# EndlessReform/smoltts

Hardware: AMD Instinct MI355X
Metric: Mimi frames/sec (=12.5 x RTF), greedy DualAR decode + Mimi decode to PCM (higher is better)
Workload: dtype bf16 weights, fp32 activations/accumulate, fp32 KV cache (LM); fp32 (Mimi)

## Files before the change

smoltts_amd/csrc/conv_xs.hip:

```cpp
#include <stdlib.h>

#include "gemm_dev.h"

namespace smoltts {

namespace {

constexpr int XS_RA_CONV = 80;
constexpr int XS_MAX_CIN = 256, XS_MAX_K_LINEAR = 512;

__device__ __forceinline__ float elu_hw_xs(float x) { return x > 0.f ? x : __expf(x) - 1.0f; }

#ifdef SMOLTTS_DBG_XS_STAMPS
__device__ unsigned long long g_xs_stamps[8 * 8];
#define XS_STAMP(I) { const long long now_ = clock64(); st_sum[I] += now_ - st_last; st_last = now_; }
#else
#define XS_STAMP(I)
#endif

template <int NTW, int MT, int RA, int EPI, int NP>
__global__ __launch_bounds__(512) void conv_xs_kernel(GemmDev p) {
  constexpr int XS_S = 16 * MT, XS_MT = MT, XS_RA = RA;
  extern __shared__ __attribute__((aligned(16))) uint4 xp[];
  const int tid = threadIdx.x, lane = tid & 63;
  const int wave = __builtin_amdgcn_readfirstlane(tid >> 6);
  const int r = lane & 15, q = lane >> 4;
  const int b = blockIdx.y, row0 = blockIdx.x * XS_S, T = p.rows_per_batch > 0 ? p.rows_per_batch : p.M;
  const int G = p.cpt * 4, nrows = XS_S + p.taps - 1, nchunks = p.K >> 5;
  const int kz = p.ksplit > 1 ? (int)blockIdx.z : 0;
  const int nt0 = (p.ksplit > 1 ? 0 : (int)blockIdx.z * 8 * NTW) + wave * NTW;
  const int nloc = p.ksplit > 1 ? p.cpt : nchunks;
  const float* xb = p.x + (long)b * p.x_bstride + (long)row0 * p.ldx + (long)kz * p.cpt * 32;
#ifdef SMOLTTS_DBG_XS_STAMPS
  long long st_sum[6] = {0, 0, 0, 0, 0, 0}, st_last = clock64();
#endif

  if (p.ln_w != nullptr) {
    float4 va[4][2];
    float* psum = reinterpret_cast<float*>(xp + 3 * G * XS_RA);
    float* stat = psum + 32 * 64;
#pragma unroll
    for (int it = 0; it < 4; ++it) {
      const int idx = tid + 512 * it, i = idx / (8 * G) * 8 + (idx & 7), g8 = (idx >> 3) % G;
      va[it][0] = va[it][1] = make_float4(0.f, 0.f, 0.f, 0.f);
      if (row0 + i < T) {
        const float* src = xb + (long)i * p.ldx + g8 * 8;
        va[it][0] = *reinterpret_cast<const float4*>(src);
        va[it][1] = *reinterpret_cast<const float4*>(src + 4);
      }
      const float4 a = va[it][0], c = va[it][1];
      psum[i * 64 + g8] = ((a.x + a.y) + (a.z + a.w)) + ((c.x + c.y) + (c.z + c.w));
    }
    lds_barrier();
    const int srow = tid >> 4, l16 = tid & 15;
    {
      const float4 t = *reinterpret_cast<const float4*>(psum + srow * 64 + l16 * 4);
      float sm = (t.x + t.y) + (t.z + t.w);
      sm += __shfl_xor(sm, 8); sm += __shfl_xor(sm, 4); sm += __shfl_xor(sm, 2); sm += __shfl_xor(sm, 1);
      if (l16 == 0) stat[srow] = sm / (float)p.K;
    }
    lds_barrier();
#pragma unroll
    for (int it = 0; it < 4; ++it) {
      const int idx = tid + 512 * it, i = idx / (8 * G) * 8 + (idx & 7), g8 = (idx >> 3) % G;
      const float mu = stat[i];
      const float4 a = va[it][0], c = va[it][1];
      float v = 0.f;
      v = fmaf(a.x - mu, a.x - mu, v); v = fmaf(a.y - mu, a.y - mu, v); v = fmaf(a.z - mu, a.z - mu, v); v = fmaf(a.w - mu, a.w - mu, v);
      v = fmaf(c.x - mu, c.x - mu, v); v = fmaf(c.y - mu, c.y - mu, v); v = fmaf(c.z - mu, c.z - mu, v); v = fmaf(c.w - mu, c.w - mu, v);
      psum[i * 64 + g8] = v;
    }
    lds_barrier();
    {
      const float4 t = *reinterpret_cast<const float4*>(psum + srow * 64 + l16 * 4);
      float sm = (t.x + t.y) + (t.z + t.w);
      sm += __shfl_xor(sm, 8); sm += __shfl_xor(sm, 4); sm += __shfl_xor(sm, 2); sm += __shfl_xor(sm, 1);
      if (l16 == 0) stat[32 + srow] = 1.0f / sqrtf(sm / (float)p.K + p.eps);
    }
    lds_barrier();
#pragma unroll
    for (int it = 0; it < 4; ++it) {
      const int idx = tid + 512 * it, i = idx / (8 * G) * 8 + (idx & 7), g8 = (idx >> 3) % G;
      const float mu = stat[i], rs = stat[32 + i];
      const float4 w0 = *reinterpret_cast<const float4*>(p.ln_w + g8 * 8), w1 = *reinterpret_cast<const float4*>(p.ln_w + g8 * 8 + 4);
      const float4 b0 = *reinterpret_cast<const float4*>(p.ln_b + g8 * 8), b1 = *reinterpret_cast<const float4*>(p.ln_b + g8 * 8 + 4);
      float4 a = va[it][0], c = va[it][1];
      a = make_float4((a.x - mu) * rs * w0.x + b0.x, (a.y - mu) * rs * w0.y + b0.y, (a.z - mu) * rs * w0.z + b0.z, (a.w - mu) * rs * w0.w + b0.w);
      c = make_float4((c.x - mu) * rs * w1.x + b1.x, (c.y - mu) * rs * w1.y + b1.y, (c.z - mu) * rs * w1.z + b1.z, (c.w - mu) * rs * w1.w + b1.w);
      uint4 h, m, l;
      split3x8(a, c, h, m, l);
      const int slot = g8 * XS_RA + i;
      xp[slot] = h;
      xp[slot + G * XS_RA] = m;
      xp[slot + 2 * G * XS_RA] = l;
    }
  } else
  for (int idx = tid; idx < ((nrows + 7) & ~7) * G; idx += 512) {
    const int i = idx / (8 * G) * 8 + (idx & 7), g8 = (idx >> 3) % G;
    if (i >= nrows) continue;
    float4 a = make_float4(0.f, 0.f, 0.f, 0.f), c = a;
    if (row0 + i < T + p.taps - 1) {
      const float* src = xb + (long)i * p.ldx + g8 * 8;
      a = *reinterpret_cast<const float4*>(src);
      c = *reinterpret_cast<const float4*>(src + 4);
    }
    if (p.pro_elu) {
      a = make_float4(elu_hw_xs(a.x), elu_hw_xs(a.y), elu_hw_xs(a.z), elu_hw_xs(a.w));
      c = make_float4(elu_hw_xs(c.x), elu_hw_xs(c.y), elu_hw_xs(c.z), elu_hw_xs(c.w));
    }
    uint4 h, m, l;
    split3x8(a, c, h, m, l);
    const int slot = g8 * XS_RA + i;
    xp[slot] = h;
    xp[slot + G * XS_RA] = m;
    xp[slot + 2 * G * XS_RA] = l;
  }

  XS_STAMP(0)
  f32x4 acc[XS_MT][NTW];
#pragma unroll
  for (int mt = 0; mt < XS_MT; ++mt)
#pragma unroll
    for (int t = 0; t < NTW; ++t) acc[mt][t] = (f32x4){0.f, 0.f, 0.f, 0.f};

  const char* wtile = p.w3 + ((size_t)nt0 * nchunks + (size_t)kz * p.cpt) * 3072;
  const int wlane = lane * 16;
  uint4 wq[2][NTW][3];
#pragma unroll
  for (int t = 0; t < NTW; ++t)
#pragma unroll
    for (int pc = 0; pc < 3; ++pc) wq[0][t][pc] = *reinterpret_cast<const uint4*>(wtile + (size_t)(t * nchunks) * 3072 + pc * 1024 + wlane);
  lds_barrier();
  XS_STAMP(1)

  int tap = 0, xc = 0;
#define XS_CHUNK(BUF, KC)                                                                                               \
  {                                                                                                                     \
    if ((KC) + 1 < nloc) {                                                                                              \
      _Pragma("unroll") for (int t = 0; t < NTW; ++t)                                                                   \
        _Pragma("unroll") for (int pc = 0; pc < 3; ++pc)                                                                \
          wq[(BUF) ^ 1][t][pc] = *reinterpret_cast<const uint4*>(wtile + (size_t)(t * nchunks + (KC) + 1) * 3072 + pc * 1024 + wlane); \
    }                                                                                                                   \
    __builtin_amdgcn_sched_barrier(0);  \
    _Pragma("unroll") for (int mt = 0; mt < XS_MT; ++mt) {                                                              \
      uint4 xf[3];                                                                                                      \
      _Pragma("unroll") for (int pc = 0; pc < 3; ++pc) xf[pc] = xp[(pc * G + xc * 4 + q) * XS_RA + mt * 16 + r + tap];  \
      _Pragma("unroll") for (int t = 0; t < NTW; ++t) acc[mt][t] = mfma_b3<NP>(wq[BUF][t], xf, acc[mt][t]);                \
    }                                                                                                                   \
    if (++xc == p.cpt) { xc = 0; ++tap; }                                                                               \
  }
  int kc = 0;
  for (; kc + 1 < nloc; kc += 2) {
    XS_CHUNK(0, kc)
    XS_CHUNK(1, kc + 1)
  }
  if (kc < nloc) XS_CHUNK(0, kc)
#undef XS_CHUNK
  XS_STAMP(2)

  if (EPI == SMOLTTS_EPI_RESID && p.ksplit <= 1 && (p.N & 15) == 0) {
    float4 rr[XS_MT][NTW];
#pragma unroll
    for (int mt = 0; mt < XS_MT; ++mt) {
      const int rl = row0 + mt * 16 + r;
#pragma unroll
      for (int t = 0; t < NTW; ++t) {
        rr[mt][t] = make_float4(0.f, 0.f, 0.f, 0.f);
        if (rl < T) rr[mt][t] = *reinterpret_cast<const float4*>(p.resid + row_off(b * T + rl, p.rows_per_batch, p.ldr, p.r_bstride) + (nt0 + t) * 16 + q * 4);
      }
    }
#pragma unroll
    for (int mt = 0; mt < XS_MT; ++mt) {
      const int rl = row0 + mt * 16 + r;
      if (rl >= T) continue;
      const long orow = row_off(b * T + rl, p.rows_per_batch, p.ldo, p.o_bstride);
#pragma unroll
      for (int t = 0; t < NTW; ++t) {
        float v[4] = {acc[mt][t][0], acc[mt][t][1], acc[mt][t][2], acc[mt][t][3]};
        rows_epilogue_resid(p, orow, (nt0 + t) * 16 + q * 4, v, rr[mt][t]);
      }
    }
  } else {
#pragma unroll
  for (int mt = 0; mt < XS_MT; ++mt) {
    const int rl = row0 + mt * 16 + r;
    if (rl >= T) continue;
    const int m = b * T + rl;
    const long orow = row_off(m, p.rows_per_batch, p.ldo, p.o_bstride);
#pragma unroll
    for (int t = 0; t < NTW; ++t) {
      const int n0 = (nt0 + t) * 16 + q * 4;
      if (p.ksplit > 1) {
        *reinterpret_cast<float4*>(p.splitk_ws + ((long)kz * p.M + m) * p.N + n0) = make_float4(acc[mt][t][0], acc[mt][t][1], acc[mt][t][2], acc[mt][t][3]);
        continue;
      }
      float v[4] = {acc[mt][t][0], acc[mt][t][1], acc[mt][t][2], acc[mt][t][3]};
      rows_epilogue<EPI>(p, m, orow, n0, v);
    }
  }
  }
#ifdef SMOLTTS_DBG_XS_STAMPS
  XS_STAMP(3)
  if (tid == 0) {
    const int st_row = p.ksplit > 1 ? 6 : (EPI == 0 && NTW == 1) ? 2 : EPI;
    for (int i = 0; i < 4; ++i) atomicAdd(&g_xs_stamps[st_row * 8 + i], (unsigned long long)st_sum[i]);
    atomicAdd(&g_xs_stamps[st_row * 8 + 6], 1ull);
  }
#endif
}

template <int NTW, int MT, int RA, int EPI, int NP>
int launch_xs_np(const GemmDev& g, int nsplit, hipStream_t stream) {
  const size_t lds = (size_t)3 * (g.cpt * 4) * RA * 16 + (g.ln_w ? (32 * 64 + 64) * sizeof(float) : 0);
  static PerDevice attr;
  const int dev = PerDevice::current();
  if (!attr.done(dev) || (int)lds > attr.value[dev]) {
    ST_CHECK_HIP(hipFuncSetAttribute((const void*)conv_xs_kernel<NTW, MT, RA, EPI, NP>, hipFuncAttributeMaxDynamicSharedMemorySize, (int)lds));
    if ((int)lds > attr.value[dev]) attr.value[dev] = (int)lds;
    attr.mark_done(dev);
  }
  const int T = g.rows_per_batch > 0 ? g.rows_per_batch : g.M;
  const dim3 grid((T + 16 * MT - 1) / (16 * MT), g.M / T, nsplit);
  hipLaunchKernelGGL((conv_xs_kernel<NTW, MT, RA, EPI, NP>), grid, dim3(512), lds, stream, g);
  ST_CHECK_HIP(hipGetLastError());
  return SMOLTTS_OK;
}

template <int NTW, int MT, int RA, int EPI>
int launch_xs(const GemmDev& g, int nsplit, hipStream_t stream) {
  return g.b3_products == 3 ? launch_xs_np<NTW, MT, RA, EPI, 3>(g, nsplit, stream) : launch_xs_np<NTW, MT, RA, EPI, 6>(g, nsplit, stream);
}

bool linear_ksplit(const GemmDev& d, int epilogue) {
  return epilogue == SMOLTTS_EPI_SCALE_RESID && d.N == 512 && d.K == 2048 && d.splitk_ws && 4L * d.M * d.N <= d.splitk_cap;
}

int linear_ntw(const GemmDev& d, int epilogue) {
  if (d.rows_per_batch > 0) {
    if (epilogue == SMOLTTS_EPI_RESID && d.K <= 256 && (d.N == 256 || d.N == 512)) return d.N / 128;
    return 0;
  }
  if (epilogue == SMOLTTS_EPI_QKV_ROPE && d.N == 1536) return 3;
  if (epilogue == SMOLTTS_EPI_SCALE_RESID && d.N == 512) return 1;
  if (epilogue == SMOLTTS_EPI_GELU && d.N == 2048) return 4;
  return 0;
}

}

bool conv_xs_applies(const GemmDev& d, int epilogue) {
  static const bool off = ST_KNOB_INT("SMOLTTS_CONV_XS", 1) == 0;
  static const bool lin_off = ST_KNOB_INT("SMOLTTS_LINEAR_XS", 1) == 0;
  if (off || !d.w3) return false;
  if (d.x_bstride % 4 != 0 || d.ldo % 4 != 0 || d.o_bstride % 4 != 0 || d.ldx % 4 != 0) return false;
  if (d.ldx >= d.K && linear_ksplit(d, epilogue)) {
    if (lin_off || d.pro_elu || d.ln_w) return false;
    const int T = d.rows_per_batch > 0 ? d.rows_per_batch : d.M;
    return d.M % T == 0 && d.M / T <= 65535 && (long)((T + 31) / 32) * (d.M / T) * 4 >= 256;
  }
  if (d.ldx >= d.K) {
    if (lin_off || d.pro_elu || d.K > XS_MAX_K_LINEAR || d.K % 32 != 0 || linear_ntw(d, epilogue) == 0) return false;
    if (d.ln_w && (d.rows_per_batch > 0 || d.K != 512 || !d.ln_b)) return false;
    if (d.rows_per_batch > 0)
      return d.M % d.rows_per_batch == 0 && d.M / d.rows_per_batch <= 65535 && (long)((d.rows_per_batch + 63) / 64) * (d.M / d.rows_per_batch) >= 256;
    return (long)((d.M + 31) / 32) * 4 >= 256;
  }
  if (d.ln_w || epilogue != SMOLTTS_EPI_STORE || d.rows_per_batch <= 0 || d.M % d.rows_per_batch != 0) return false;
  if (d.ldx % 32 != 0 || d.ldx > XS_MAX_CIN || d.K % d.ldx != 0) return false;
  const int taps = (int)(d.K / d.ldx);
  if (taps < 2 || 64 + taps - 1 > XS_RA_CONV || (d.N != 128 && d.N != 640)) return false;
  const long tiles = (long)((d.rows_per_batch + 63) / 64) * (d.M / d.rows_per_batch);
  return tiles >= 256 && d.M / d.rows_per_batch <= 65535;
}

int launch_conv_xs(const GemmDev& d, int epilogue, hipStream_t stream) {
  GemmDev g = d;
  if (d.ldx >= d.K && linear_ksplit(d, epilogue)) {
    g.taps = 1;
    g.cpt = 16;
    g.ksplit = 4;
    ST_TRY((launch_xs<4, 2, 32, SMOLTTS_EPI_SCALE_RESID>(g, 4, stream)));
    hipLaunchKernelGGL((splitk_reduce_kernel<SMOLTTS_EPI_SCALE_RESID>), dim3((unsigned)(((long)d.M * (d.N >> 2) + 255) / 256)), dim3(256), 0, stream, g);
    ST_CHECK_HIP(hipGetLastError());
    return SMOLTTS_OK;
  }
  if (d.ldx >= d.K) {
    g.taps = 1;
    g.cpt = d.K >> 5;
    if (d.rows_per_batch > 0)
      return d.N == 256 ? launch_xs<2, 4, 64, SMOLTTS_EPI_RESID>(g, 1, stream) : launch_xs<4, 4, 64, SMOLTTS_EPI_RESID>(g, 1, stream);
    switch (linear_ntw(d, epilogue)) {
      case 3: return launch_xs<3, 2, 32, SMOLTTS_EPI_QKV_ROPE>(g, 4, stream);
      case 1: return launch_xs<1, 2, 32, SMOLTTS_EPI_SCALE_RESID>(g, 4, stream);
      default: return launch_xs<4, 2, 32, SMOLTTS_EPI_GELU>(g, 4, stream);
    }
  }
  g.taps = (int)(d.K / d.ldx);
  g.cpt = (int)(d.ldx >> 5);
  return d.N == 640 ? launch_xs<5, 4, XS_RA_CONV, SMOLTTS_EPI_STORE>(g, 1, stream) : launch_xs<1, 4, XS_RA_CONV, SMOLTTS_EPI_STORE>(g, 1, stream);
}

}

#ifdef SMOLTTS_DBG_XS_STAMPS
extern "C" int smoltts_debug_xs_stamps(unsigned long long* out64, int reset) {
  if (hipMemcpyFromSymbol(out64, HIP_SYMBOL(smoltts::g_xs_stamps), 64 * sizeof(unsigned long long)) != hipSuccess) return -1;
  if (reset) {
    unsigned long long z[64] = {0};
    if (hipMemcpyToSymbol(HIP_SYMBOL(smoltts::g_xs_stamps), z, sizeof(z)) != hipSuccess) return -1;
  }
  return 0;
}
#endif
```

Before: 28550.

## Replace split-K linear plus reduce kernel with intra-block K-parts reduction

```diff
diff --git a/smoltts_amd/csrc/conv_xs.hip b/smoltts_amd/csrc/conv_xs.hip
--- a/smoltts_amd/csrc/conv_xs.hip
+++ b/smoltts_amd/csrc/conv_xs.hip
@@ -27,10 +27,9 @@
   const int r = lane & 15, q = lane >> 4;
   const int b = blockIdx.y, row0 = blockIdx.x * XS_S, T = p.rows_per_batch > 0 ? p.rows_per_batch : p.M;
   const int G = p.cpt * 4, nrows = XS_S + p.taps - 1, nchunks = p.K >> 5;
-  const int kz = p.ksplit > 1 ? (int)blockIdx.z : 0;
-  const int nt0 = (p.ksplit > 1 ? 0 : (int)blockIdx.z * 8 * NTW) + wave * NTW;
-  const int nloc = p.ksplit > 1 ? p.cpt : nchunks;
-  const float* xb = p.x + (long)b * p.x_bstride + (long)row0 * p.ldx + (long)kz * p.cpt * 32;
+  const int nt0 = (int)blockIdx.z * 8 * NTW + wave * NTW;
+  const int nloc = nchunks;
+  const float* xb = p.x + (long)b * p.x_bstride + (long)row0 * p.ldx;
 #ifdef SMOLTTS_DBG_XS_STAMPS
   long long st_sum[6] = {0, 0, 0, 0, 0, 0}, st_last = clock64();
 #endif
@@ -123,7 +122,7 @@
 #pragma unroll
     for (int t = 0; t < NTW; ++t) acc[mt][t] = (f32x4){0.f, 0.f, 0.f, 0.f};
 
-  const char* wtile = p.w3 + ((size_t)nt0 * nchunks + (size_t)kz * p.cpt) * 3072;
+  const char* wtile = p.w3 + (size_t)nt0 * nchunks * 3072;
   const int wlane = lane * 16;
   uint4 wq[2][NTW][3];
 #pragma unroll
@@ -158,7 +157,7 @@
 #undef XS_CHUNK
   XS_STAMP(2)
 
-  if (EPI == SMOLTTS_EPI_RESID && p.ksplit <= 1 && (p.N & 15) == 0) {
+  if (EPI == SMOLTTS_EPI_RESID && (p.N & 15) == 0) {
     float4 rr[XS_MT][NTW];
 #pragma unroll
     for (int mt = 0; mt < XS_MT; ++mt) {
@@ -190,10 +189,6 @@
 #pragma unroll
     for (int t = 0; t < NTW; ++t) {
       const int n0 = (nt0 + t) * 16 + q * 4;
-      if (p.ksplit > 1) {
-        *reinterpret_cast<float4*>(p.splitk_ws + ((long)kz * p.M + m) * p.N + n0) = make_float4(acc[mt][t][0], acc[mt][t][1], acc[mt][t][2], acc[mt][t][3]);
-        continue;
-      }
       float v[4] = {acc[mt][t][0], acc[mt][t][1], acc[mt][t][2], acc[mt][t][3]};
       rows_epilogue<EPI>(p, m, orow, n0, v);
     }
@@ -202,7 +197,7 @@
 #ifdef SMOLTTS_DBG_XS_STAMPS
   XS_STAMP(3)
   if (tid == 0) {
-    const int st_row = p.ksplit > 1 ? 6 : (EPI == 0 && NTW == 1) ? 2 : EPI;
+    const int st_row = (EPI == 0 && NTW == 1) ? 2 : EPI;
     for (int i = 0; i < 4; ++i) atomicAdd(&g_xs_stamps[st_row * 8 + i], (unsigned long long)st_sum[i]);
     atomicAdd(&g_xs_stamps[st_row * 8 + 6], 1ull);
   }
@@ -231,8 +226,139 @@
   return g.b3_products == 3 ? launch_xs_np<NTW, MT, RA, EPI, 3>(g, nsplit, stream) : launch_xs_np<NTW, MT, RA, EPI, 6>(g, nsplit, stream);
 }
 
-bool linear_ksplit(const GemmDev& d, int epilogue) {
-  return epilogue == SMOLTTS_EPI_SCALE_RESID && d.N == 512 && d.K == 2048 && d.splitk_ws && 4L * d.M * d.N <= d.splitk_cap;
+constexpr int KP_PARTS = 4, KP_CPP = 16, KP_SL = 4;
+constexpr int KP_RED_LD = 132;
+
+template <int NP>
+__global__ __launch_bounds__(512) void linear_kparts_kernel(GemmDev p) {
+  constexpr int RA = 32, G = KP_PARTS * KP_SL * 4, NTW = 4, MT = 2;
+  extern __shared__ __attribute__((aligned(16))) uint4 xp[];
+  const int tid = threadIdx.x, lane = tid & 63;
+  const int wave = __builtin_amdgcn_readfirstlane(tid >> 6);
+  const int r = lane & 15, q = lane >> 4;
+  const int kz = wave >> 1, half = wave & 1;
+  const int b = blockIdx.y, row0 = blockIdx.x * 32, T = p.rows_per_batch > 0 ? p.rows_per_batch : p.M;
+  const int nchunks = KP_PARTS * KP_CPP;
+  const int nt0 = (int)blockIdx.z * 8 + half * NTW;
+  const float* xb = p.x + (long)b * p.x_bstride + (long)row0 * p.ldx;
+
+  float4 va[4][2];
+  auto fetch_x = [&](int s) {
+#pragma unroll
+    for (int it = 0; it < 4; ++it) {
+      const int idx = tid + 512 * it, i = idx / (8 * G) * 8 + (idx & 7), g8 = (idx >> 3) % G;
+      const int lc = g8 >> 2, kc = (lc >> 2) * KP_CPP + s * KP_SL + (lc & 3);
+      va[it][0] = va[it][1] = make_float4(0.f, 0.f, 0.f, 0.f);
+      if (row0 + i < T) {
+        const float* src = xb + (long)i * p.ldx + kc * 32 + (g8 & 3) * 8;
+        va[it][0] = *reinterpret_cast<const float4*>(src);
+        va[it][1] = *reinterpret_cast<const float4*>(src + 4);
+      }
+    }
+  };
+  auto store_x = [&]() {
+#pragma unroll
+    for (int it = 0; it < 4; ++it) {
+      const int idx = tid + 512 * it, i = idx / (8 * G) * 8 + (idx & 7), g8 = (idx >> 3) % G;
+      uint4 h, m, l;
+      split3x8(va[it][0], va[it][1], h, m, l);
+      const int slot = g8 * RA + i;
+      xp[slot] = h;
+      xp[slot + G * RA] = m;
+      xp[slot + 2 * G * RA] = l;
+    }
+  };
+  fetch_x(0);
+
+  f32x4 acc[MT][NTW];
+#pragma unroll
+  for (int mt = 0; mt < MT; ++mt)
+#pragma unroll
+    for (int t = 0; t < NTW; ++t) acc[mt][t] = (f32x4){0.f, 0.f, 0.f, 0.f};
+
+  const char* wtile = p.w3 + ((size_t)nt0 * nchunks + (size_t)kz * KP_CPP) * 3072;
+  const int wlane = lane * 16;
+  uint4 wq[2][NTW][3];
+#pragma unroll
+  for (int t = 0; t < NTW; ++t)
+#pragma unroll
+    for (int pc = 0; pc < 3; ++pc) wq[0][t][pc] = *reinterpret_cast<const uint4*>(wtile + (size_t)(t * nchunks) * 3072 + pc * 1024 + wlane);
+  store_x();
+  lds_barrier();
+
+#define KP_CHUNK(BUF, J, C)                                                                                             \
+  {                                                                                                                     \
+    if ((J) + 1 < KP_CPP) {                                                                                             \
+      _Pragma("unroll") for (int t = 0; t < NTW; ++t)                                                                   \
+        _Pragma("unroll") for (int pc = 0; pc < 3; ++pc)                                                                \
+          wq[(BUF) ^ 1][t][pc] = *reinterpret_cast<const uint4*>(wtile + (size_t)(t * nchunks + (J) + 1) * 3072 + pc * 1024 + wlane); \
+    }                                                                                                                   \
+    __builtin_amdgcn_sched_barrier(0);                                  \
+    _Pragma("unroll") for (int mt = 0; mt < MT; ++mt) {                                                                 \
+      uint4 xf[3];                                                                                                      \
+      _Pragma("unroll") for (int pc = 0; pc < 3; ++pc) xf[pc] = xp[(pc * G + (kz * KP_SL + (C)) * 4 + q) * RA + mt * 16 + r]; \
+      _Pragma("unroll") for (int t = 0; t < NTW; ++t) acc[mt][t] = mfma_b3<NP>(wq[BUF][t], xf, acc[mt][t]);             \
+    }                                                                                                                   \
+  }
+  for (int s = 0; s < KP_CPP / KP_SL; ++s) {
+    const bool more = s + 1 < KP_CPP / KP_SL;
+    if (more) fetch_x(s + 1);
+    const int j = s * KP_SL;
+    KP_CHUNK(0, j, 0)
+    KP_CHUNK(1, j + 1, 1)
+    KP_CHUNK(0, j + 2, 2)
+    KP_CHUNK(1, j + 3, 3)
+    lds_barrier();
+    if (more) {
+      store_x();
+      lds_barrier();
+    }
+  }
+#undef KP_CHUNK
+
+  float* red = reinterpret_cast<float*>(xp);
+#pragma unroll
+  for (int mt = 0; mt < MT; ++mt)
+#pragma unroll
+    for (int t = 0; t < NTW; ++t)
+      *reinterpret_cast<float4*>(red + (kz * 32 + mt * 16 + r) * KP_RED_LD + (half * NTW + t) * 16 + q * 4) =
+          make_float4(acc[mt][t][0], acc[mt][t][1], acc[mt][t][2], acc[mt][t][3]);
+  lds_barrier();
+#pragma unroll
+  for (int it = 0; it < 2; ++it) {
+    const int idx = tid + 512 * it, row = idx >> 5, c4 = idx & 31;
+    const int rl = row0 + row;
+    if (rl >= T) continue;
+    float v[4] = {0.f, 0.f, 0.f, 0.f};
+#pragma unroll
+    for (int s = 0; s < KP_PARTS; ++s) {
+      const float4 t = *reinterpret_cast<const float4*>(red + (s * 32 + row) * KP_RED_LD + c4 * 4);
+      v[0] += t.x; v[1] += t.y; v[2] += t.z; v[3] += t.w;
+    }
+    const int m = b * T + rl;
+    rows_epilogue<SMOLTTS_EPI_SCALE_RESID>(p, m, row_off(m, p.rows_per_batch, p.ldo, p.o_bstride), (int)blockIdx.z * 128 + c4 * 4, v);
+  }
+}
+
+template <int NP>
+int launch_kparts_np(const GemmDev& g, hipStream_t stream) {
+  constexpr int lds = 3 * (KP_PARTS * KP_SL * 4) * 32 * 16;
+  static_assert(KP_PARTS * 32 * KP_RED_LD * (int)sizeof(float) <= lds, "the partial tiles reuse the piece planes");
+  static PerDevice attr;
+  const int dev = PerDevice::current();
+  if (!attr.done(dev)) {
+    ST_CHECK_HIP(hipFuncSetAttribute((const void*)linear_kparts_kernel<NP>, hipFuncAttributeMaxDynamicSharedMemorySize, lds));
+    attr.mark_done(dev);
+  }
+  const int T = g.rows_per_batch > 0 ? g.rows_per_batch : g.M;
+  const dim3 grid((T + 31) / 32, g.M / T, 4);
+  hipLaunchKernelGGL((linear_kparts_kernel<NP>), grid, dim3(512), lds, stream, g);
+  ST_CHECK_HIP(hipGetLastError());
+  return SMOLTTS_OK;
+}
+
+bool linear_kparts(const GemmDev& d, int epilogue) {
+  return epilogue == SMOLTTS_EPI_SCALE_RESID && d.N == 512 && d.K == KP_PARTS * KP_CPP * 32;
 }
 
 int linear_ntw(const GemmDev& d, int epilogue) {
@@ -253,7 +379,7 @@
   static const bool lin_off = ST_KNOB_INT("SMOLTTS_LINEAR_XS", 1) == 0;
   if (off || !d.w3) return false;
   if (d.x_bstride % 4 != 0 || d.ldo % 4 != 0 || d.o_bstride % 4 != 0 || d.ldx % 4 != 0) return false;
-  if (d.ldx >= d.K && linear_ksplit(d, epilogue)) {
+  if (d.ldx >= d.K && linear_kparts(d, epilogue)) {
     if (lin_off || d.pro_elu || d.ln_w) return false;
     const int T = d.rows_per_batch > 0 ? d.rows_per_batch : d.M;
     return d.M % T == 0 && d.M / T <= 65535 && (long)((T + 31) / 32) * (d.M / T) * 4 >= 256;
@@ -275,15 +401,8 @@
 
 int launch_conv_xs(const GemmDev& d, int epilogue, hipStream_t stream) {
   GemmDev g = d;
-  if (d.ldx >= d.K && linear_ksplit(d, epilogue)) {
-    g.taps = 1;
-    g.cpt = 16;
-    g.ksplit = 4;
-    ST_TRY((launch_xs<4, 2, 32, SMOLTTS_EPI_SCALE_RESID>(g, 4, stream)));
-    hipLaunchKernelGGL((splitk_reduce_kernel<SMOLTTS_EPI_SCALE_RESID>), dim3((unsigned)(((long)d.M * (d.N >> 2) + 255) / 256)), dim3(256), 0, stream, g);
-    ST_CHECK_HIP(hipGetLastError());
-    return SMOLTTS_OK;
-  }
+  if (d.ldx >= d.K && linear_kparts(d, epilogue))
+    return d.b3_products == 3 ? launch_kparts_np<3>(g, stream) : launch_kparts_np<6>(g, stream);
   if (d.ldx >= d.K) {
     g.taps = 1;
     g.cpt = d.K >> 5;
```

Result: no change. 28600 (median of 6 runs) (+0.2%).
